# revdotcom/paper_accurate_fast_cheap

Measured on AMD Instinct MI355X. Metric: audio-sec/sec (1/RTF) GigaSpeech long-form encode, higher is better.
Workload: dtype f32+bf16-slot

## Files before the change

### include/pafc_encoder_ops.h

```cpp
#ifndef PAFC_ENCODER_OPS_H
#define PAFC_ENCODER_OPS_H

#include "pafc_wkv6.h"

#ifdef __cplusplus
extern "C" {
#endif

int pafc_dwconv1d_cl(int dtype, int B, int T_in, int C, int K, int left_pad, int T_out, const void *x,
                     const void *w, const void *bias, void *y, int glu, const int32_t *lens,
                     pafc_stream_t stream);

int pafc_dwconv1d_cl_ex(int dtype, int B, int T_in, int C, int K, int left_pad, int T_out, const void *x, long ldx,
                        const void *w, const void *bias, void *y, int act, const int32_t *lens, pafc_stream_t stream);

int pafc_dwconv1d_cl_ln_silu(int dtype, int B, int T_in, int C, int K, int left_pad, int T_out, const void *x, long ldx,
                             const void *w, const void *bias, const void *gamma, const void *beta, float eps, void *y,
                             const int32_t *lens, pafc_stream_t stream);

size_t pafc_dwconv1d_cl_wgrad_workspace_bytes(int B, int T_out, int C, int K);
int pafc_dwconv1d_cl_wgrad(int dtype, int B, int T_in, int C, int K, int left_pad, int T_out, const void *x, long ldx,
                           const void *dy, float *dw, float *dbias, void *workspace, size_t workspace_bytes,
                           pafc_stream_t stream);

int pafc_add_layernorm(int dtype, int dtype_out, int rows, int C, const void *x, const void *y, float alpha,
                       const int32_t *lens, int T, int mask_y, void *x_out, const void *gamma1, const void *beta1,
                       void *out1, long ld1, int silu1, int zero1, const void *gamma2, const void *beta2, void *out2,
                       long ld2, float eps, pafc_stream_t stream);

int pafc_add_layernorm_ex(int dtype, int dtype_out, int dtype_out2, int rows, int C, const void *x, const void *y, float alpha,
                          const int32_t *lens, int T, int mask_y, void *x_out, const void *gamma1, const void *beta1,
                          void *out1, long ld1, int silu1, int zero1, const void *gamma2, const void *beta2, void *out2,
                          long ld2, float eps, float *stats_x, float *stats_out1, pafc_stream_t stream);
int pafc_gemm_bf16_ph_ln(long M, int N, int K, const void *A, long lda, const void *W, long ldw, const void *bias,
                         const void *residual, long ldr, void *out, long ldo, float alpha, int act, int ln_mode, float *stats,
                         const float *csum, int ln_c, float ln_eps, int tile_m, pafc_stream_t stream);

int pafc_split_planes(long rows, int cols, const float *x, long ldx, void *out, long ldo, long lo_off, int triple,
                      pafc_stream_t stream);

size_t pafc_layernorm_bwd_workspace_bytes(long rows, int C);
int pafc_layernorm_bwd(int dtype_x, int dtype_dy, long rows, int C, const void *x, const void *dy, const void *gamma,
                       float eps, void *dx, float *dgamma_dbeta, void *workspace, size_t workspace_bytes,
                       pafc_stream_t stream);
int pafc_layernorm_bwd_add(int dtype_x, int dtype_dy, long rows, int C, const void *x, const void *dy, const void *gamma, float eps,
                           const void *dx_add, void *dx, float *dgamma_dbeta, void *workspace, size_t workspace_bytes,
                           pafc_stream_t stream);
// ... 183 lines not shown
```

### paper_accurate_fast_cheap_amd/_lib.py

```python
import ctypes
import os
from ctypes import c_float, c_int, c_long, c_size_t, c_ulonglong, c_void_p

import torch

_HERE = os.path.dirname(os.path.abspath(__file__))
SO_PATH = os.path.join(_HERE, "libpafc_hip.so")

PAFC_F32, PAFC_BF16 = 0, 1
_ERRORS = {
    -1: "null pointer", -2: "bad dims (B, T, C, H must be positive and C == H * 64)", -3: "head size must be 64",
    -4: "workspace too small", -5: "kernel launch failed", -6: "unsupported dtype", -7: "unsupported",
    -8: "r, k, v, w, y must be 16-byte aligned",
}


class PafcError(RuntimeError):
    pass


_lib = None


def lib():
# ... 12 lines not shown
            "(python -m paper_accurate_fast_cheap_amd.csrc.build). There is no CPU fallback.")
    from .csrc import build as _build
    if _build.built_key() != _build.source_key():
        raise PafcError(
            f"{SO_PATH} was not built from the sources in this tree (libpafc_hip.so.json: {_build.built_key()}, sources: "
            f"{_build.source_key()}): rebuild with python -m paper_accurate_fast_cheap_amd.csrc.build")
    _lib = _bind(ctypes.CDLL(SO_PATH))
    return _lib


P, I, G, Z, F, U = c_void_p, c_int, c_long, c_size_t, c_float, c_ulonglong
SIGNATURES = {
    "pafc_mha_rows": (I, [I, I, I, I, P, G, P, P, G, P, P, P, I, P, G, P]),
    "pafc_logp_gather_rows": (I, [I, G, I, P, G, P, P, P]),
    "pafc_mha_band": (I, [I, I, I, I, I, I, I, P, G, P, P, G, P, G, P, P, P, G, P]),
    "pafc_mha_rows_lse": (I, [I, I, I, I, P, G, P, P, G, P, P, P, I, P, G, P, P]),
    "pafc_mha_rows_bwd_workspace_bytes": (Z, [G, I]),
    "pafc_mha_rows_bwd": (I, [I, I, I, I, G, P, G, P, P, G, P, G, P, G, P, P, P, P, I, P, G, P, P, G, P, Z, P]),
    "pafc_lsm_loss_rows": (I, [I, G, I, P, G, P, F, P, P, P, P]),
    "pafc_lsm_loss_rows_bwd": (I, [I, G, I, P, G, P, F, P, P, P, G, P]),
    "pafc_mha_band_lse": (I, [I, I, I, I, I, I, I, P, G, P, P, G, P, G, P, P, P, G, P, P]),
    "pafc_mha_band_bwd_workspace_bytes": (Z, [I, I, I]),
    "pafc_mha_band_bwd": (I, [I, I, I, I, I, I, I, P, G, P, P, G, P, G, P, P, P, G, P, G, P, P, G, P, P, G, P, G, P, P, P, Z,
                              P]),
    "pafc_mha_step": (I, [I, I, I, I, I, I, P, G, P, P, P, P, P, G, P]),
    "pafc_attn_beam_select_workspace_bytes": (Z, [I, I]),
    "pafc_attn_beam_select": (I, [I, I, I, I, I, I, I, P, G, P, P, P, P, P, P, P, P, P, P, Z, P]),
    "pafc_mha_step_paths": (I, [I, I, I, I, I, I, P, G, P, P, G, P, P, P, P, G, P]),
    "pafc_joint_candidates": (I, [I, I, I, I, I, I, F, P, P, P, P, P, P, P]),
    "pafc_joint_frame": (I, [P, I, I, I, P, G, P, P, I, P]),
    "pafc_joint_collect": (I, [P, P, P, P, P, P, P, P]),
    "pafc_dwconv1d_cl": (I, [I, I, I, I, I, I, I, P, P, P, P, I, P, P]),
    "pafc_dwconv1d_cl_ex": (I, [I, I, I, I, I, I, I, P, G, P, P, P, I, P, P]),
    "pafc_dwconv1d_cl_ln_silu": (I, [I, I, I, I, I, I, I, P, G, P, P, P, P, F, P, P, P]),
    "pafc_dwconv1d_cl_wgrad_workspace_bytes": (Z, [I, I, I, I]),
    "pafc_dwconv1d_cl_wgrad": (I, [I, I, I, I, I, I, I, P, G, P, P, P, P, Z, P]),
    "pafc_add_layernorm": (I, [I, I, I, I, P, P, F, P, I, I, P, P, P, P, G, I, I, P, P, P, G, F, P]),
    "pafc_add_layernorm_ex": (I, [I, I, I, I, I, P, P, F, P, I, I, P, P, P, P, G, I, I, P, P, P, G, F, P, P, P]),
    "pafc_gemm_bf16_ph_ln": (I, [G, I, I, P, G, P, G, P, P, G, P, G, F, I, I, P, P, I, F, I, P]),
    "pafc_split_planes": (I, [G, I, P, G, P, G, G, I, P]),
    "pafc_layernorm_bwd_workspace_bytes": (Z, [G, I]),
    "pafc_layernorm_bwd": (I, [I, I, G, I, P, P, P, F, P, P, P, Z, P]),
    "pafc_layernorm_bwd_add": (I, [I, I, G, I, P, P, P, F, P, P, P, P, Z, P]),
    "pafc_layernorm_silu_fwd": (I, [I, I, G, I, P, P, P, F, P, P]),
    "pafc_layernorm_silu_bwd": (I, [I, I, G, I, P, P, P, P, F, P, P, P, Z, P]),
    "pafc_gemm_skinny_bf16": (I, [G, I, I, I, P, G, G, P, G, G, P, G, P, G, G, P, G, G, F, I, P, I, P, F, P, P]),
    "pafc_gemm_skinny_bf16_ex": (I, [G, I, I, I, P, G, G, P, G, G, P, G, P, G, G, P, G, G, F, I, I, P, I, I, P, F, P, P, P, I,
        P, P, F, P]),
    "pafc_decay_lora_skinny_bf16": (I, [G, I, I, P, G, P, P, P, P, G, P]),
    "pafc_tmix_shift_mix": (I, [I, I, I, I, I, I, P, P, P, P, P]),
    "pafc_tmix_mix4": (I, [I, I, I, I, I, I, P, P, P, P, P]),
    "pafc_tmix_lora_mix4_bf16": (I, [I, I, I, I, I, P, P, P, P, P, P]),
    "pafc_tmix_lora_down_bf16": (I, [I, I, I, I, I, I, P, P, P, P, P]),
    "pafc_tmix_shift_mix_prev": (I, [I, I, I, I, I, I, P, P, P, P, P, P]),
    "pafc_tmix_lora_mix4_bf16_prev": (I, [I, I, I, I, I, P, P, P, P, P, P, P]),
    "pafc_tmix_lora_down_bf16_prev": (I, [I, I, I, I, I, I, P, P, P, P, P, P]),
    "pafc_decay_lora_bf16": (I, [G, I, I, I, P, P, P, P, P, P]),
    "pafc_tmix_bwd_workspace_bytes": (Z, [G, I]),
    "pafc_tmix_shift_mix_bwd": (I, [I, I, I, I, I, P, P, P, P, P, P, Z, P]),
    "pafc_tmix_mix4_bwd": (I, [I, I, I, I, I, P, P, P, P, P, P, P, P, P, P, P, Z, P]),
    "pafc_tmix_mix4_bwd_rows": (I, [I, I, I, I, I, P, P, P, P, P, P, P, P, P, P, P, Z, P]),
    "pafc_conv3x3s2_nhwc_bf16": (I, [I, I, I, I, I, P, P, P, P, I, P]),
    "pafc_conv3x3s2_c1_nhwc_bf16": (I, [I, I, I, I, P, P, P, P, I, P]),
    "pafc_conv3x3s2_c1_wgrad_workspace_bytes": (Z, [I, I, I]),
    "pafc_conv3x3s2_c1_wgrad_bf16": (I, [I, I, I, I, P, P, P, P, P, Z, P]),
    "pafc_conv3x3s2_c1_nhwc_f32split": (I, [I, I, I, I, P, P, P, P, P, I, P]),
# ... 154 lines not shown
```

### paper_accurate_fast_cheap_amd/csrc/dwconv.hip

```cpp
#include <stdlib.h>
#include "pafc_common.h"
#include "../../include/pafc_encoder_ops.h"

namespace pafc {
namespace {

constexpr int KMAX = 31;
constexpr int TO = 16;

template <typename ET> struct Pair;
template <> struct Pair<float> {
    __device__ static __forceinline__ float2 load(const float *p) { return *reinterpret_cast<const float2 *>(p); }
    __device__ static __forceinline__ void store(float *p, float2 v) { *reinterpret_cast<float2 *>(p) = v; }
    __device__ static __forceinline__ float round(float v) { return v; }
};
template <> struct Pair<bf16_t> {
    __device__ static __forceinline__ float2 load(const bf16_t *p) {
        const uint32_t q = *reinterpret_cast<const uint32_t *>(p);
        return make_float2(bf16_bits_to_f32(q & 0xffffu), __uint_as_float(q & 0xffff0000u));
    }
    __device__ static __forceinline__ void store(bf16_t *p, float2 v) {
        *reinterpret_cast<uint32_t *>(p) = f32_to_bf16_bits(v.x) | (f32_to_bf16_bits(v.y) << 16);
    }
    __device__ static __forceinline__ float round(float v) { return round_bf16(v); }
};

__device__ __forceinline__ float sigmoidf_(float x) { return 1.f / (1.f + __expf(-x)); }

struct LnTail {
    const void *gamma, *beta;
    float eps;
};

// ... 85 lines not shown
        const float inv_c = 1.f / (float)C;
        float mean[TO];
#pragma unroll
        for (int o = 0; o < TO; ++o) {
            mean[o] = tot[o] * inv_c;
            const float d0 = u0[o] - mean[o], d1 = u1[o] - mean[o];
            sv[o] = fmaf(d1, d1, d0 * d0);
        }
        __syncthreads();
        block_sums(sv);
        const float2 gv = Pair<ET>::load((const ET *)ln.gamma + c), bt = Pair<ET>::load((const ET *)ln.beta + c);
#pragma unroll
        for (int o = 0; o < TO; ++o) {
            const float rstd = rsqrtf(tot[o] * inv_c + ln.eps);
            float o0 = Pair<ET>::round(fmaf((u0[o] - mean[o]) * rstd, gv.x, bt.x));
            float o1 = Pair<ET>::round(fmaf((u1[o] - mean[o]) * rstd, gv.y, bt.y));
            o0 = o0 * sigmoidf_(o0);
            o1 = o1 * sigmoidf_(o1);
            if (t0 + o < T_out) Pair<ET>::store(yb + (size_t)(t0 + o) * C, make_float2(o0, o1));
        }
        return;
    }
#pragma unroll
    for (int o = 0; o < TO; ++o) {
        if (ACT == 2) {
            const float u0 = Pair<ET>::round(a0[o]), u1 = Pair<ET>::round(a1[o]);
            a0[o] = u0 * sigmoidf_(u0);
            a1[o] = u1 * sigmoidf_(u1);
        }
        if (t0 + o < T_out) Pair<ET>::store(yb + (size_t)(t0 + o) * C, make_float2(a0[o], a1[o]));
    }
}

template <typename ET, int K>
int launch(int B, int T_in, int C, int left_pad, int T_out, const void *x, long ldx, const void *w, const void *bias,
           void *y, int act, const int32_t *lens, const LnTail &ln, hipStream_t s) {
    dim3 grid((T_out + TO - 1) / TO, (C / 2 + 255) / 256, B), block(256);
    if (act == 1)
        hipLaunchKernelGGL((dwconv_kernel<ET, K, 1>), grid, block, 0, s, T_in, C, left_pad, T_out, (const ET *)x, ldx,
                           (const ET *)w, (const ET *)bias, (ET *)y, lens, ln);
    else if (act == 2)
        hipLaunchKernelGGL((dwconv_kernel<ET, K, 2>), grid, block, 0, s, T_in, C, left_pad, T_out, (const ET *)x, ldx,
                           (const ET *)w, (const ET *)bias, (ET *)y, lens, ln);
    else if (act == 3) {
        if constexpr (K == 31 || K == 15) {
            hipLaunchKernelGGL((dwconv_kernel<ET, K, 3>), grid, block, 0, s, T_in, C, left_pad, T_out, (const ET *)x, ldx,
                               (const ET *)w, (const ET *)bias, (ET *)y, lens, ln);
        } else {
            return PAFC_ERR_UNSUPPORTED;
        }
    } else
        hipLaunchKernelGGL((dwconv_kernel<ET, K, 0>), grid, block, 0, s, T_in, C, left_pad, T_out, (const ET *)x, ldx,
                           (const ET *)w, (const ET *)bias, (ET *)y, lens, ln);
    return hipGetLastError() == hipSuccess ? PAFC_OK : PAFC_ERR_LAUNCH;
}

template <typename ET>
int dispatch_k(int K, int B, int T_in, int C, int left_pad, int T_out, const void *x, long ldx, const void *w,
               const void *bias, void *y, int act, const int32_t *lens, const LnTail &ln, hipStream_t s) {
    switch (K) {
        case 31: return launch<ET, 31>(B, T_in, C, left_pad, T_out, x, ldx, w, bias, y, act, lens, ln, s);
        case 15: return launch<ET, 15>(B, T_in, C, left_pad, T_out, x, ldx, w, bias, y, act, lens, ln, s);
        case 7: return launch<ET, 7>(B, T_in, C, left_pad, T_out, x, ldx, w, bias, y, act, lens, ln, s);
        case 4: return launch<ET, 4>(B, T_in, C, left_pad, T_out, x, ldx, w, bias, y, act, lens, ln, s);
        case 3: return launch<ET, 3>(B, T_in, C, left_pad, T_out, x, ldx, w, bias, y, act, lens, ln, s);
        default: return PAFC_ERR_UNSUPPORTED;
    }
}


constexpr int WG_SPAN = 8 * TO;

template <typename ET, int K>
__global__ __launch_bounds__(256) void dwconv_wgrad_kernel(int T_in, int C, int left_pad, int T_out,
                                                           const ET *__restrict__ x, long ldx,
                                                           const ET *__restrict__ dy, float *__restrict__ part) {
    const int c = (blockIdx.y * 256 + threadIdx.x) * 2;
    if (c >= C) return;
    const int b = blockIdx.z;
    const ET *xb = x + (size_t)b * T_in * ldx;
    const ET *db = dy + (size_t)b * T_out * C;
    float a0[K], a1[K], s0 = 0.f, s1 = 0.f;
#pragma unroll
    for (int k = 0; k < K; ++k) a0[k] = a1[k] = 0.f;
    constexpr int NR = TO + K - 1;
    for (int t0 = blockIdx.x * WG_SPAN; t0 < min(T_out, (int)(blockIdx.x + 1) * WG_SPAN); t0 += TO) {
        float2 g[TO], in[NR];
#pragma unroll
        for (int o = 0; o < TO; ++o) {
            const int t = min(t0 + o, T_out - 1);
            g[o] = Pair<ET>::load(db + (size_t)t * C + c);
            if (t0 + o >= T_out) g[o] = make_float2(0.f, 0.f);
            s0 += g[o].x;
            s1 += g[o].y;
        }
#pragma unroll
        for (int q = 0; q < NR; ++q) {
            const int s = t0 - left_pad + q;
// ... 42 lines not shown
    return hipGetLastError() == hipSuccess ? PAFC_OK : PAFC_ERR_LAUNCH;
}

template <typename ET>
int dispatch_wgrad(int K, int B, int T_in, int C, int left_pad, int T_out, const void *x, long ldx, const void *dy,
                   float *part, float *dw, float *dbias, hipStream_t s) {
    switch (K) {
        case 31: return launch_wgrad<ET, 31>(B, T_in, C, left_pad, T_out, x, ldx, dy, part, dw, dbias, s);
        case 15: return launch_wgrad<ET, 15>(B, T_in, C, left_pad, T_out, x, ldx, dy, part, dw, dbias, s);
        case 7: return launch_wgrad<ET, 7>(B, T_in, C, left_pad, T_out, x, ldx, dy, part, dw, dbias, s);
        case 4: return launch_wgrad<ET, 4>(B, T_in, C, left_pad, T_out, x, ldx, dy, part, dw, dbias, s);
        case 3: return launch_wgrad<ET, 3>(B, T_in, C, left_pad, T_out, x, ldx, dy, part, dw, dbias, s);
        default: return PAFC_ERR_UNSUPPORTED;
    }
}

}
}

extern "C" int pafc_dwconv1d_cl(int dtype, int B, int T_in, int C, int K, int left_pad, int T_out, const void *x,
                                const void *w, const void *bias, void *y, int glu, const int32_t *lens,
                                pafc_stream_t stream) {
    if (!x || !w || !y) return PAFC_ERR_NULL_POINTER;
    if (B <= 0 || T_in <= 0 || T_out <= 0 || C <= 0 || (C % 2) || K <= 0 || K > pafc::KMAX || left_pad < 0 ||
        B > 65535)
        return PAFC_ERR_BAD_DIMS;
    return pafc_dwconv1d_cl_ex(dtype, B, T_in, C, K, left_pad, T_out, x, glu ? 2L * C : (long)C, w, bias, y, glu ? 1 : 0, lens,
                               stream);
}

extern "C" int pafc_dwconv1d_cl_ex(int dtype, int B, int T_in, int C, int K, int left_pad, int T_out, const void *x, long ldx,
                                   const void *w, const void *bias, void *y, int act, const int32_t *lens,
                                   pafc_stream_t stream) {
    if (!x || !w || !y) return PAFC_ERR_NULL_POINTER;
    if (B <= 0 || T_in <= 0 || T_out <= 0 || C <= 0 || (C % 2) || K <= 0 || K > pafc::KMAX || left_pad < 0 ||
        B > 65535 || act < 0 || act > 2 || ldx < (act == 1 ? 2L * C : (long)C) || (ldx % 2))
        return PAFC_ERR_BAD_DIMS;
    hipStream_t s = (hipStream_t)stream;
    const pafc::LnTail none{nullptr, nullptr, 0.f};
    if (dtype == PAFC_BF16)
        return pafc::dispatch_k<pafc::bf16_t>(K, B, T_in, C, left_pad, T_out, x, ldx, w, bias, y, act, lens, none, s);
    if (dtype == PAFC_F32) return pafc::dispatch_k<float>(K, B, T_in, C, left_pad, T_out, x, ldx, w, bias, y, act, lens, none, s);
    return PAFC_ERR_DTYPE;
}

extern "C" int pafc_dwconv1d_cl_ln_silu(int dtype, int B, int T_in, int C, int K, int left_pad, int T_out, const void *x, long ldx,
                                        const void *w, const void *bias, const void *gamma, const void *beta, float eps, void *y,
                                        const int32_t *lens, pafc_stream_t stream) {
    if (!x || !w || !y || !gamma || !beta) return PAFC_ERR_NULL_POINTER;
    if (B <= 0 || T_in <= 0 || T_out <= 0 || left_pad < 0 || B > 65535 || ldx < C || (ldx % 2)) return PAFC_ERR_BAD_DIMS;
    if (C != 512 || (K != 31 && K != 15)) return PAFC_ERR_UNSUPPORTED;
    if (dtype != PAFC_BF16) return PAFC_ERR_DTYPE;
    const pafc::LnTail ln{gamma, beta, eps};
    return pafc::dispatch_k<pafc::bf16_t>(K, B, T_in, C, left_pad, T_out, x, ldx, w, bias, y, 3, lens, ln, (hipStream_t)stream);
}

extern "C" size_t pafc_dwconv1d_cl_wgrad_workspace_bytes(int B, int T_out, int C, int K) {
    if (B <= 0 || T_out <= 0 || C <= 0 || K <= 0) return 0;
    return (size_t)B * ((T_out + pafc::WG_SPAN - 1) / pafc::WG_SPAN) * (K + 1) * C * sizeof(float);
}

extern "C" int pafc_dwconv1d_cl_wgrad(int dtype, int B, int T_in, int C, int K, int left_pad, int T_out, const void *x,
                                      long ldx, const void *dy, float *dw, float *dbias, void *workspace,
                                      size_t workspace_bytes, pafc_stream_t stream) {
    if (!x || !dy || !dw || !workspace) return PAFC_ERR_NULL_POINTER;
    if (B <= 0 || T_in <= 0 || T_out <= 0 || C <= 0 || (C % 2) || K <= 0 || K > pafc::KMAX || left_pad < 0 ||
        B > 65535 || ldx < C || (ldx % 2))
        return PAFC_ERR_BAD_DIMS;
    if (workspace_bytes < pafc_dwconv1d_cl_wgrad_workspace_bytes(B, T_out, C, K)) return PAFC_ERR_WORKSPACE;
    hipStream_t s = (hipStream_t)stream;
    float *part = (float *)workspace;
    if (dtype == PAFC_BF16)
        return pafc::dispatch_wgrad<pafc::bf16_t>(K, B, T_in, C, left_pad, T_out, x, ldx, dy, part, dw, dbias, s);
    if (dtype == PAFC_F32) return pafc::dispatch_wgrad<float>(K, B, T_in, C, left_pad, T_out, x, ldx, dy, part, dw, dbias, s);
    return PAFC_ERR_DTYPE;
}
```

### paper_accurate_fast_cheap_amd/hip_ops.py

```python
import contextlib
import ctypes
import math
import os
import threading
import weakref
from typing import List, Optional

import torch

from . import _lib
from ._lib import c_int, c_void_p
from .utils import graph_step


DISPATCH = dict(skinny_max_rows=640, own_gemm_min_rows=1, lds_resident_min_rows=8192, split_gemm_min_rows=1024,
                ln_fold_min_rows=24576, dwconv_ln_silu_max_rows=24575, split_small_max_rows=8192, split_layers_min_rows=256,
                ktail_min_k=2048)


def _load_dispatch():
    legacy = dict(skinny_max_rows="PAFC_SKINNY_MAX_ROWS", own_gemm_min_rows="PAFC_OWN_GEMM_MIN_ROWS",
                  lds_resident_min_rows="PAFC_LDS_RESIDENT_MIN_ROWS", split_gemm_min_rows="PAFC_SPLIT_GEMM_MIN_ROWS")
    for name, env in legacy.items():
        if os.environ.get(env):
            DISPATCH[name] = int(os.environ[env])
    for item in filter(None, os.environ.get("PAFC_DISPATCH", "").split(",")):
        name, _, value = item.partition("=")
        if name.strip() not in DISPATCH:
            raise ValueError(f"PAFC_DISPATCH: unknown threshold {name!r} (known: {sorted(DISPATCH)})")
        DISPATCH[name.strip()] = int(value)


_load_dispatch()


def train_gemms_own() -> bool:
    return os.environ.get("PAFC_TRAIN_OWN_GEMMS", "1") != "0"


def train_kernels_enabled() -> bool:
    import os
    return os.environ.get("PAFC_TRAIN_KERNELS", "1") != "0"


def _conv_rows_ld(x: torch.Tensor, who: str) -> int:
    if not x.is_cuda:
        raise _lib.PafcError("this op runs on the MI355X only (tensor is on %s); there is no CPU fallback" % x.device)
    if x.is_contiguous():
        return x.shape[-1]
    if x.dim() != 3 or x.stride(2) != 1 or x.stride(0) != x.shape[1] * x.stride(1) or x.stride(1) < x.shape[2] or x.stride(1) % 2 \
            or x.data_ptr() % (2 * x.element_size()):
        raise _lib.PafcError(f"{who}: x (B, T, C) with unit channel stride, rows of one even stride, an aligned channel pair")
    return x.stride(1)


def depthwise_conv1d_cl(x: torch.Tensor, weight: torch.Tensor, bias: Optional[torch.Tensor], left_pad: int,
                        out_len: int, glu: bool = False, lens: Optional[torch.Tensor] = None) -> torch.Tensor:
    _lib.require_gpu(weight, bias, lens)
    ldx = _conv_rows_ld(x, "depthwise_conv1d_cl")
    B, T, Cx = x.shape
    C = Cx // 2 if glu else Cx
    K = weight.shape[-1]
    if weight.shape != (C, 1, K) or weight.dtype != x.dtype or (bias is not None and bias.dtype != x.dtype):
        raise _lib.PafcError("depthwise weight must be (C, 1, K) in the activation dtype")
    if lens is not None and lens.dtype != torch.int32:
        raise _lib.PafcError("lens must be int32")
    y = torch.empty(B, out_len, C, dtype=x.dtype, device=x.device)
    rc = _lib.lib().pafc_dwconv1d_cl_ex(_lib.dtype_code(x.dtype), B, T, C, K, left_pad, out_len, _lib.ptr(x), ldx,
                                        _lib.ptr(weight), _lib.ptr(bias), _lib.ptr(y), int(glu), _lib.ptr(lens),
                                        _lib.stream_of(x))
    _lib.check(rc, "pafc_dwconv1d_cl")
    return y


def dwconv_ln_silu_ok(x: torch.Tensor, weight: torch.Tensor) -> bool:
    return (x.numel() // x.shape[-1] <= DISPATCH["dwconv_ln_silu_max_rows"] and x.dtype == torch.bfloat16 and x.is_cuda
            and x.shape[-1] == 512 and weight.shape[-1] in (15, 31))


def depthwise_conv1d_cl_ln_silu(x: torch.Tensor, weight: torch.Tensor, bias: Optional[torch.Tensor], left_pad: int, out_len: int,
                                gamma: torch.Tensor, beta: torch.Tensor, eps: float, lens: Optional[torch.Tensor] = None):
    _lib.require_gpu(weight, bias, gamma, beta, lens)
    ldx = _conv_rows_ld(x, "depthwise_conv1d_cl_ln_silu")
    B, T, C = x.shape
    K = weight.shape[-1]
    if not dwconv_ln_silu_ok(x, weight) or weight.shape != (C, 1, K) or any(
            t is not None and (t.dtype != x.dtype or not t.is_contiguous()) for t in (weight, bias, gamma, beta)):
        raise _lib.PafcError("depthwise_conv1d_cl_ln_silu: bf16, C = 512, K in (15, 31), contiguous parameters in the activation dtype")
    if lens is not None and lens.dtype != torch.int32:
        raise _lib.PafcError("lens must be int32")
    L = _lib.lib()
    y = torch.empty(B, out_len, C, dtype=x.dtype, device=x.device)
    rc = L.pafc_dwconv1d_cl_ln_silu(_lib.dtype_code(x.dtype), B, T, C, K, left_pad, out_len, _lib.ptr(x), ldx, _lib.ptr(weight),
                                    _lib.ptr(bias), _lib.ptr(gamma), _lib.ptr(beta), float(eps), _lib.ptr(y), _lib.ptr(lens),
                                    _lib.stream_of(x))
    _lib.check(rc, "pafc_dwconv1d_cl_ln_silu")
    return y


def depthwise_conv1d_cl_wgrad(x: torch.Tensor, dy: torch.Tensor, K: int, left_pad: int, want_bias: bool = True):
    _lib.require_gpu(dy)
    ldx = _conv_rows_ld(x, "depthwise_conv1d_cl_wgrad")
# ... 3488 lines not shown
```

### paper_accurate_fast_cheap_amd/transformer/fused.py

```python
from typing import List, Optional, Tuple

import os

import torch
import torch.nn.functional as F
from torch import nn

from .. import hip_ops
from ..rwkv_v6.rwkv_wrapper import RWKV_TmixWrapper
from ..rwkv_v6.rwkv_wrapper_bidirectional import RWKV_TmixWrapper_bidirectional
from ..rwkv_v6.rwkv_wrapper_bidirectional_direction_dropout import (RWKV_TmixWrapper_bidirectional_direction_dropout,
                                                                     RWKV_TmixWrapper_bidirectional_direction_dropout_both)
from ..rwkv_v6.wkv6_op import wkv6_forward, wkv6_forward_bidir


_DIR_DROP_SLOTS = (RWKV_TmixWrapper_bidirectional_direction_dropout, RWKV_TmixWrapper_bidirectional_direction_dropout_both)
_RWKV_SLOTS = (RWKV_TmixWrapper, RWKV_TmixWrapper_bidirectional) + _DIR_DROP_SLOTS


def _fold_norm(w: torch.Tensor, b: Optional[torch.Tensor], norm: nn.LayerNorm, interleave: int = 0):
    wf = w.float()
    bf = (b.float() if b is not None else 0) + wf @ norm.bias.float()
    wp = (wf * norm.weight.float()).to(torch.bfloat16)
    if interleave:
# ... 10 lines not shown
        self.rwkv = type(slot) in _RWKV_SLOTS
        self.reverse0 = False
        if type(slot) in _DIR_DROP_SLOTS:
            fwd, bwd = slot.rwkv_wrapper_forward, slot.rwkv_wrapper_backward
            if slot.bi_active:
                self.blocks = [fwd.tmix_block, bwd.tmix_block]
            elif slot.alt_decoding and slot.layer_id % 2 == 1:
                self.blocks, self.reverse0 = [bwd.tmix_block], True
            else:
                self.blocks = [fwd.tmix_block]
            self.slot_bf16 = bool(fwd.do_bfloat16)
        elif isinstance(slot, RWKV_TmixWrapper_bidirectional):
            self.blocks = [slot.rwkv_wrapper_forward.tmix_block, slot.rwkv_wrapper_backward.tmix_block]
        elif self.rwkv:
            self.blocks = [slot.tmix_block]
        else:
            self.blocks = []
        self.ndir = len(self.blocks)
        if type(slot) not in _DIR_DROP_SLOTS:
            self.slot_bf16 = bool(getattr(slot, "do_bfloat16", False))
        self._stamp = None
        self.refresh()

    def _current_stamp(self):
        ep = hip_ops.param_epoch()
        if getattr(self, "_stamp_params", None) is None or self._stamp_epoch != ep:
            L = self.layer
            ps = [p for b in self.blocks for p in b.parameters()] + [L.feed_forward_macaron.w_2.bias, L.feed_forward.w_2.bias,
                                                                        L.conv_module.pointwise_conv1.weight,
                                                                        L.conv_module.pointwise_conv1.bias,
                                                                        L.feed_forward_macaron.w_1.weight, L.feed_forward_macaron.w_2.weight,
                                                                        L.feed_forward.w_1.weight, L.feed_forward.w_2.weight,
                                                                        L.conv_module.pointwise_conv2.weight,
                                                                        L.norm_ff_macaron.weight, L.norm_ff_macaron.bias, L.norm_ff.weight,
                                                                        L.norm_ff.bias, L.norm_conv.weight, L.norm_conv.bias,
                                                                        L.feed_forward_macaron.w_1.bias, L.feed_forward.w_1.bias]
            self._stamp_params = [p for p in ps if p is not None]
            self._stamp_epoch = ep
        return (ep,) + tuple((p.data_ptr(), p._version, p.dtype) for p in self._stamp_params)

    def refresh(self):
        stamp = self._current_stamp()
        if stamp == self._stamp:
            self._fill.use()
            return
        bl = self.blocks
        with torch.no_grad():
            if self.rwkv:
                self._refresh_rwkv(bl)
            L = self.layer
            self.b2_macaron = (L.feed_forward_macaron.w_2.bias * L.ff_scale).contiguous()
            self.b2 = (L.feed_forward.w_2.bias * L.ff_scale).contiguous()
            pw1 = L.conv_module.pointwise_conv1
            self.pw1_glu = None
            rows2 = pw1.weight.shape[0]
            if pw1.weight.dtype == torch.bfloat16 and pw1.weight.is_cuda and rows2 % 128 == 0 \
                    and pw1.weight.shape[1] % 64 == 0:
                self.pw1_glu = {h: (hip_ops.glu_interleave(pw1.weight.squeeze(-1), h),
                                    hip_ops.glu_interleave(pw1.bias, h) if pw1.bias is not None else None)
                                for h in ((64, 32) if rows2 % 256 == 0 else (64,))}
            self._refresh_split()
            self._refresh_lnfold()
        self._stamp = stamp
        self._fill = hip_ops.DerivedFill()

    def _refresh_lnfold(self):
        L = self.layer
        self.lnf = None
        w1 = L.feed_forward.w_1.weight
        cm = L.conv_module
        if not (self.rwkv and w1.dtype == torch.bfloat16 and w1.is_cuda and L.size == 512 and L.feed_forward_macaron is not None
                and cm is not None and cm.pointwise_conv1.weight.shape[0] % 256 == 0 and cm.lorder == 0
                and os.environ.get("PAFC_LN_FOLD", "1") != "0"):
            return
        pw1 = cm.pointwise_conv1
        self.lnf = dict(ffm=_fold_norm(L.feed_forward_macaron.w_1.weight, L.feed_forward_macaron.w_1.bias, L.norm_ff_macaron),
                        ff=_fold_norm(L.feed_forward.w_1.weight, L.feed_forward.w_1.bias, L.norm_ff),
                        pw1=_fold_norm(pw1.weight.squeeze(-1), pw1.bias, L.norm_conv, interleave=32))

    def carry_folds(self):
        if getattr(self, "_carry_folds", None) is not None and self._carry_folds[0] == self._stamp:
            self._carry_folds[2].use()
            return self._carry_folds[1]
        L = self.layer
        folds = dict(ff=_fold_norm(L.feed_forward.w_1.weight, L.feed_forward.w_1.bias, L.norm_ff) + (L.norm_ff.eps,))
        if self.rwkv:
            folds["out"] = _fold_norm(self.Wo, None, self.blocks[0].ln_x) + (self.blocks[0].ln_x.eps,)
        self._carry_folds = (self._stamp, folds, hip_ops.DerivedFill())
        return folds

    def _refresh_split(self):
        L = self.layer
        self.split = None
        w1 = L.feed_forward.w_1.weight
        cm = L.conv_module
        if not (self.rwkv and self.slot_bf16 and w1.dtype == torch.float32 and w1.is_cuda and L.size % 128 == 0
                and w1.shape[0] % 128 == 0 and cm is not None and cm.pointwise_conv1.weight.shape[0] % 256 == 0):
            return
        sp = hip_ops.split_planes
        pw1 = cm.pointwise_conv1
        self.split = dict(
            ffm_w1=sp(L.feed_forward_macaron.w_1.weight.contiguous(), True), ffm_w2=sp(L.feed_forward_macaron.w_2.weight.contiguous(), True),
            ff_w1=sp(L.feed_forward.w_1.weight.contiguous(), True), ff_w2=sp(L.feed_forward.w_2.weight.contiguous(), True),
            pw1=sp(hip_ops.glu_interleave(pw1.weight.squeeze(-1), 32).contiguous(), True),
            pw1_b=hip_ops.glu_interleave(pw1.bias, 32).contiguous() if pw1.bias is not None else None,
            pw1_plain=sp(pw1.weight.squeeze(-1).contiguous(), True),
            pw2=sp(cm.pointwise_conv2.weight.squeeze(-1).contiguous(), True))

    def _refresh_rwkv(self, bl):
        self.maa_x = [b.time_maa_x.reshape(-1).contiguous() for b in bl]
        self.maa_x_n = torch.stack(self.maa_x).contiguous()
        self.W1 = torch.stack([b.time_maa_rkvw_w1 for b in bl]).contiguous()
        self.W1n = torch.stack([b.time_maa_rkvw_w1.t() for b in bl]).contiguous()
        self.D1n = torch.stack([b.time_decay_w1.t() for b in bl]).contiguous()
        self.W2 = [b.time_maa_rkvw_w2.contiguous() for b in bl]
        self.W2t = torch.stack([b.time_maa_rkvw_w2.transpose(1, 2) for b in bl]).contiguous()
        self.maa4 = torch.stack([torch.stack([b.time_maa_r.reshape(-1), b.time_maa_k.reshape(-1),
                                              b.time_maa_v.reshape(-1), b.time_maa_w.reshape(-1)])
                                 for b in bl]).contiguous()
        self.Wrkv = torch.stack([getattr(b, n).weight.t() for n in ("receptance", "key", "value") for b in bl]
                                ).contiguous()
        self.Wrkv_n = torch.stack([getattr(b, n).weight for n in ("receptance", "key", "value") for b in bl]
                                  ).contiguous()
        self.D2n = torch.stack([b.time_decay_w2.t() for b in bl]).contiguous()
        self.D1 = torch.stack([b.time_decay_w1 for b in bl]).contiguous()
        self.D2 = torch.stack([b.time_decay_w2 for b in bl]).contiguous()
        self.time_decay = torch.stack([b.time_decay.reshape(1, -1) for b in bl]).contiguous()
        self.u = [b.time_faaaa.contiguous() for b in bl]
        wo = torch.cat([b.output.weight for b in bl], dim=1)
        self.Wo = (wo * 0.5 if self.ndir == 2 else wo).contiguous()


def _layer_shape_common(layer: nn.Module) -> bool:
    cm = layer.conv_module
    return (layer.normalize_before and layer.feed_forward_macaron is not None and cm is not None
            and cm.use_layer_norm and isinstance(cm.activation, nn.SiLU)
            and isinstance(layer.feed_forward.activation, nn.SiLU)
            and isinstance(layer.feed_forward_macaron.activation, nn.SiLU))


# ... 225 lines not shown
    xo = x2.view(B, T, C)
    if next_fold:
        stn = new_stats()
        return _ln(L.norm_final, xo, want_x=False, stats_out1=stn)[1], stn
    return _final_norms(L, xo, next_norm)


_SPLIT_GEMM_MIN_ROWS = hip_ops.DISPATCH["split_layers_min_rows"]


def split_eligible(plan: LayerPlan, x: torch.Tensor) -> bool:
    return (plan.split is not None and x.dtype == torch.float32 and x.is_cuda
            and x.numel() // x.shape[-1] >= _SPLIT_GEMM_MIN_ROWS)


def layer_forward_split(plan: LayerPlan, x: torch.Tensor, hp: torch.Tensor, lens: Optional[torch.Tensor],
                        next_norm: Optional[nn.LayerNorm], next_split: bool):
    L, S = plan.layer, plan.split
    B, T, C = x.shape
    M = B * T
    masked = lens is not None
    cm = L.conv_module
    G = hip_ops.gemm_ph_ex
    x = _ffn_split(L.feed_forward_macaron, S["ffm_w1"], S["ffm_w2"], hp, x, L.ff_scale, plan.b2_macaron, inplace=False)
    h = _ln(L.norm_mha, x, out_dtype=torch.bfloat16, want_x=False)[1]
    x = slot_forward(plan, h, residual=x)
    hc = _ln(L.norm_conv, x, zero_rows=masked, lens=lens, T=T, want_x=False, split1=True)[1]
    hc, left_pad, Tc = _causal_pad(cm, hc, T)
    if B * Tc <= hip_ops._SPLIT_SMALL_MAX_ROWS and B * Tc * 2 * C <= (1 << 22):
        p = G(hc.view(B * Tc, 2 * C), S["pw1_plain"], cm.pointwise_conv1.bias, a_split=True, out_kind="f32").view(B, Tc, 2 * C)
        dw = hip_ops.depthwise_conv1d_cl(p, cm.depthwise_conv.weight, cm.depthwise_conv.bias, left_pad, T, glu=True)
    else:
        p = G(hc.view(B * Tc, 2 * C), S["pw1"], S["pw1_b"], "glu", a_split=True, out_kind="f32").view(B, Tc, C)
        dw = hip_ops.depthwise_conv1d_cl(p, cm.depthwise_conv.weight, cm.depthwise_conv.bias, left_pad, T)
    g = _ln(cm.norm, dw, silu=True, split1=True)[1]
    if not masked:
        x2 = x.view(M, C)
        G(g.view(M, 2 * C), S["pw2"], cm.pointwise_conv2.bias, residual=x2, out=x2, a_split=True, out_kind="f32")
        h2 = _ln(L.norm_ff, x, want_x=False, split1=True)[1]
    else:
        c = G(g.view(M, 2 * C), S["pw2"], cm.pointwise_conv2.bias, a_split=True, out_kind="f32").view(B, T, C)
        x, h2, _ = _ln(L.norm_ff, x, c, lens=lens, T=T, mask_y=True, split1=True)
    x = _ffn_split(L.feed_forward, S["ff_w1"], S["ff_w2"], h2, x, L.ff_scale, plan.b2, inplace=True)
    return _final_norms(L, x, next_norm, split_next=next_split)


def _carry_slot_ok(slot: nn.Module) -> bool:
    if type(slot) is RWKV_TmixWrapper:
        return bool(slot.do_bfloat16)
    from .mamba2 import MambaAttWrapper
    if type(slot) is MambaAttWrapper and slot.streamable:
        m = slot.mamba
        return bool(m.fused_inference and m.ssd_kernel and m.d_state == 128 and m.d_inner <= 1024
                    and m.conv1d.weight.dtype == torch.bfloat16 and m.in_proj.weight.dtype == torch.bfloat16)
    return False


def carry_eligible(layer: nn.Module, x: torch.Tensor) -> bool:
    cm = layer.conv_module
    return (_layer_shape_common(layer) and _carry_slot_ok(layer.self_attn) and cm.lorder > 0 and cm.kernel_size <= 31
            and layer.size % 64 == 0 and layer.size <= 1024 and x.is_cuda and x.dtype == torch.bfloat16)


def _chunk_slot_rwkv(plan: LayerPlan, h: torch.Tensor, x: torch.Tensor, shift: torch.Tensor, s_in: Optional[torch.Tensor], *,
                     sk: bool, in_place: bool, out: Optional[torch.Tensor] = None):
    B, T, C = h.shape
    M = B * T
# ... 221 lines not shown
```

Before: 48830.

## Add persistent software-pipelined f32 depthwise conv kernel with transposed taps

Adds a persistent depthwise-conv kernel for f32 K=31 with no activation. Each block loops over strided time tiles and prefetches the next tile's input rows into registers while computing the current one. The grid is sized to the CU count, and tiles are partitioned into groups. Weights can be supplied pre-transposed as (K, C), which allows coalesced float2 tap loads; the layer plan caches this transpose. The large register footprint (31 taps ×2 plus 46 rows of float2) risks spills or low occupancy, and the kernel is enabled by default, with an env var to turn it off.

```diff
diff --git a/include/pafc_encoder_ops.h b/include/pafc_encoder_ops.h
--- a/include/pafc_encoder_ops.h
+++ b/include/pafc_encoder_ops.h
@@ -13,6 +13,10 @@
 
 int pafc_dwconv1d_cl_ex(int dtype, int B, int T_in, int C, int K, int left_pad, int T_out, const void *x, long ldx,
                         const void *w, const void *bias, void *y, int act, const int32_t *lens, pafc_stream_t stream);
+
+int pafc_dwconv1d_cl_tw(int dtype, int B, int T_in, int C, int K, int left_pad, int T_out, const void *x, long ldx,
+                        const void *w, const void *wt, const void *bias, void *y, int act, const int32_t *lens,
+                        pafc_stream_t stream);
 
 int pafc_dwconv1d_cl_ln_silu(int dtype, int B, int T_in, int C, int K, int left_pad, int T_out, const void *x, long ldx,
                              const void *w, const void *bias, const void *gamma, const void *beta, float eps, void *y,
diff --git a/paper_accurate_fast_cheap_amd/_lib.py b/paper_accurate_fast_cheap_amd/_lib.py
--- a/paper_accurate_fast_cheap_amd/_lib.py
+++ b/paper_accurate_fast_cheap_amd/_lib.py
@@ -68,6 +68,7 @@
     "pafc_joint_collect": (I, [P, P, P, P, P, P, P, P]),
     "pafc_dwconv1d_cl": (I, [I, I, I, I, I, I, I, P, P, P, P, I, P, P]),
     "pafc_dwconv1d_cl_ex": (I, [I, I, I, I, I, I, I, P, G, P, P, P, I, P, P]),
+    "pafc_dwconv1d_cl_tw": (I, [I, I, I, I, I, I, I, P, G, P, P, P, P, I, P, P]),
     "pafc_dwconv1d_cl_ln_silu": (I, [I, I, I, I, I, I, I, P, G, P, P, P, P, F, P, P, P]),
     "pafc_dwconv1d_cl_wgrad_workspace_bytes": (Z, [I, I, I, I]),
     "pafc_dwconv1d_cl_wgrad": (I, [I, I, I, I, I, I, I, P, G, P, P, P, P, Z, P]),
diff --git a/paper_accurate_fast_cheap_amd/csrc/dwconv.hip b/paper_accurate_fast_cheap_amd/csrc/dwconv.hip
--- a/paper_accurate_fast_cheap_amd/csrc/dwconv.hip
+++ b/paper_accurate_fast_cheap_amd/csrc/dwconv.hip
@@ -1,4 +1,5 @@
 #include <stdlib.h>
+#include <type_traits>
 #include "pafc_common.h"
 #include "../../include/pafc_encoder_ops.h"
 
@@ -150,9 +151,142 @@
     }
 }
 
+__device__ __forceinline__ float2 dw_load_row(const float *xb, long xc, int c, int T_in, int s) {
+    const int sc = min(max(s, 0), T_in - 1);
+    return Pair<float>::load(xb + (size_t)sc * xc + c);
+}
+
+template <int K, int NPF, bool WT>
+__global__ __launch_bounds__(256, 2) void dwconv_pipe_kernel(int T_in, int C, int left_pad, int T_out, const float *__restrict__ x,
+                                                             long ldx, const float *__restrict__ w, const float *__restrict__ wt,
+                                                             const float *__restrict__ bias, float *__restrict__ y,
+                                                             const int32_t *__restrict__ lens, int groups) {
+    constexpr int NR = TO + K - 1, NA = NPF;
+    static_assert(NPF >= 0 && NPF <= NR, "rows ahead");
+    const int c = (blockIdx.y * 256 + threadIdx.x) * 2;
+    if (c >= C) return;
+    const int b = blockIdx.z;
+    const int ntiles = (T_out + TO - 1) / TO;
+    const int grp = blockIdx.x % groups, stride = ((int)gridDim.x - grp + groups - 1) / groups;
+    const int hi = (int)((long)ntiles * (grp + 1) / groups);
+    int tile = (int)((long)ntiles * grp / groups) + blockIdx.x / groups;
+    if (tile >= hi) return;
+    const float *xb = x + (size_t)b * T_in * ldx;
+    float *yb = y + (size_t)b * T_out * C + c;
+    const int valid = lens ? min(T_in, lens[b]) : T_in;
+
+    float w0[K], w1[K];
+    if constexpr (WT) {
+#pragma unroll
+        for (int k = 0; k < K; ++k) {
+            const float2 t = Pair<float>::load(wt + (size_t)k * C + c);
+            w0[k] = t.x;
+            w1[k] = t.y;
+        }
+    } else {
+#pragma unroll
+        for (int k = 0; k < K; ++k) {
+            w0[k] = w[(size_t)c * K + k];
+            w1[k] = w[(size_t)(c + 1) * K + k];
+        }
+    }
+    float2 bv = make_float2(0.f, 0.f);
+    if (bias) bv = Pair<float>::load(bias + c);
+
+    float2 in[NR];
+#pragma unroll
+    for (int q = 0; q < NR; ++q) in[q] = dw_load_row(xb, ldx, c, T_in, tile * TO - left_pad + q);
+
+    auto body = [&](auto has_next) {
+        constexpr bool NEXT = decltype(has_next)::value;
+        const int t0 = tile * TO, s0 = t0 - left_pad, n0 = s0 + stride * TO;
+        auto row = [&](int q) {
+            const int s = s0 + q;
+            return (s >= 0 && s < valid) ? in[q] : make_float2(0.f, 0.f);
+        };
+        float2 ahead[NA > 0 ? NA : 1];
+        if constexpr (NEXT && NA > 0) {
+#pragma unroll
+            for (int q = 0; q < NA; ++q) {
+                ahead[q] = row(q);
+                in[q] = dw_load_row(xb, ldx, c, T_in, n0 + q);
+                __builtin_amdgcn_sched_barrier(0);
+            }
+        }
+        float a0[TO], a1[TO];
+#pragma unroll
+        for (int o = 0; o < TO; ++o) { a0[o] = bv.x; a1[o] = bv.y; }
+#pragma unroll
+        for (int q = 0; q < NR; ++q) {
+            const float2 v = (NEXT && q < NA) ? ahead[q] : row(q);
+#pragma unroll
+            for (int o = 0; o < TO; ++o) {
+                const int k = q - o;
+                if (k >= 0 && k < K) {
+                    a0[o] = fmaf(w0[k], v.x, a0[o]);
+                    a1[o] = fmaf(w1[k], v.y, a1[o]);
+                }
+            }
+        }
+        if constexpr (NEXT) {
+#pragma unroll
+            for (int q = NA; q < NR; ++q) in[q] = dw_load_row(xb, ldx, c, T_in, n0 + q);
+            __builtin_amdgcn_sched_barrier(0);
+        }
+        if constexpr (!NEXT) {
+#pragma unroll
+            for (int o = 0; o < TO; ++o) asm volatile("" : "+v"(a0[o]), "+v"(a1[o]));
+        }
+#pragma unroll
+        for (int o = 0; o < TO; ++o)
+            if (NEXT || t0 + o < T_out) Pair<float>::store(yb + (size_t)(t0 + o) * C, make_float2(a0[o], a1[o]));
+    };
+    if (tile + stride < hi) {
+        __builtin_amdgcn_s_waitcnt(0x0F70);
+        do {
+            body(std::true_type{});
+            tile += stride;
+        } while (tile + stride < hi);
+    }
+    body(std::false_type{});
+}
+
+bool dwconv_pipe() {
+    const char *e = getenv("PAFC_DWCONV_PIPE");
+    return !(e && e[0] == '0');
+}
+
+constexpr int PIPE_ROWS_AHEAD = 28;
+constexpr int PIPE_BLOCKS_PER_CU = 2;
+
+template <int K>
+int launch_pipe(int B, int T_in, int C, int left_pad, int T_out, const float *x, long ldx, const float *w, const float *wt,
+                const float *bias, float *y, const int32_t *lens, hipStream_t s) {
+    const int ntiles = (T_out + TO - 1) / TO, ycols = (C / 2 + 255) / 256;
+    long nblk = (long)device_cus() * PIPE_BLOCKS_PER_CU / ((long)B * ycols);
+    if (const char *e = getenv("PAFC_DWCONV_BLOCKS")) nblk = atol(e);
+    nblk = nblk < 1 ? 1 : (nblk > ntiles ? ntiles : nblk);
+    dim3 grid((unsigned)nblk, ycols, B), block(256);
+    int groups = nblk < 8 ? (int)nblk : 8;
+    if (const char *e = getenv("PAFC_DWCONV_GROUPS")) groups = atoi(e) < 1 ? 1 : (atoi(e) < nblk ? atoi(e) : (int)nblk);
+#define PAFC_DWPIPE_(NPF, WT) \
+    hipLaunchKernelGGL((dwconv_pipe_kernel<K, NPF, WT>), grid, block, 0, s, T_in, C, left_pad, T_out, x, ldx, w, wt, bias, y, lens, \
+                       groups)
+    if (wt) PAFC_DWPIPE_(PIPE_ROWS_AHEAD, true); else PAFC_DWPIPE_(PIPE_ROWS_AHEAD, false);
+#undef PAFC_DWPIPE_
+    return hipGetLastError() == hipSuccess ? PAFC_OK : PAFC_ERR_LAUNCH;
+}
+
 template <typename ET, int K>
-int launch(int B, int T_in, int C, int left_pad, int T_out, const void *x, long ldx, const void *w, const void *bias,
+int launch(int B, int T_in, int C, int left_pad, int T_out, const void *x, long ldx, const void *w, const void *wt, const void *bias,
            void *y, int act, const int32_t *lens, const LnTail &ln, hipStream_t s) {
+    if constexpr (sizeof(ET) == 4 && K == 31) {
+        if (act == 0) {
+            if (dwconv_pipe())
+                return launch_pipe<K>(B, T_in, C, left_pad, T_out, (const float *)x, ldx, (const float *)w, (const float *)wt,
+                                      (const float *)bias, (float *)y, lens, s);
+        }
+    }
     dim3 grid((T_out + TO - 1) / TO, (C / 2 + 255) / 256, B), block(256);
     if (act == 1)
         hipLaunchKernelGGL((dwconv_kernel<ET, K, 1>), grid, block, 0, s, T_in, C, left_pad, T_out, (const ET *)x, ldx,
@@ -174,14 +308,14 @@
 }
 
 template <typename ET>
-int dispatch_k(int K, int B, int T_in, int C, int left_pad, int T_out, const void *x, long ldx, const void *w,
+int dispatch_k(int K, int B, int T_in, int C, int left_pad, int T_out, const void *x, long ldx, const void *w, const void *wt,
                const void *bias, void *y, int act, const int32_t *lens, const LnTail &ln, hipStream_t s) {
     switch (K) {
-        case 31: return launch<ET, 31>(B, T_in, C, left_pad, T_out, x, ldx, w, bias, y, act, lens, ln, s);
-        case 15: return launch<ET, 15>(B, T_in, C, left_pad, T_out, x, ldx, w, bias, y, act, lens, ln, s);
-        case 7: return launch<ET, 7>(B, T_in, C, left_pad, T_out, x, ldx, w, bias, y, act, lens, ln, s);
-        case 4: return launch<ET, 4>(B, T_in, C, left_pad, T_out, x, ldx, w, bias, y, act, lens, ln, s);
-        case 3: return launch<ET, 3>(B, T_in, C, left_pad, T_out, x, ldx, w, bias, y, act, lens, ln, s);
+        case 31: return launch<ET, 31>(B, T_in, C, left_pad, T_out, x, ldx, w, wt, bias, y, act, lens, ln, s);
+        case 15: return launch<ET, 15>(B, T_in, C, left_pad, T_out, x, ldx, w, wt, bias, y, act, lens, ln, s);
+        case 7: return launch<ET, 7>(B, T_in, C, left_pad, T_out, x, ldx, w, wt, bias, y, act, lens, ln, s);
+        case 4: return launch<ET, 4>(B, T_in, C, left_pad, T_out, x, ldx, w, wt, bias, y, act, lens, ln, s);
+        case 3: return launch<ET, 3>(B, T_in, C, left_pad, T_out, x, ldx, w, wt, bias, y, act, lens, ln, s);
         default: return PAFC_ERR_UNSUPPORTED;
     }
 }
@@ -290,15 +424,22 @@
 extern "C" int pafc_dwconv1d_cl_ex(int dtype, int B, int T_in, int C, int K, int left_pad, int T_out, const void *x, long ldx,
                                    const void *w, const void *bias, void *y, int act, const int32_t *lens,
                                    pafc_stream_t stream) {
+    return pafc_dwconv1d_cl_tw(dtype, B, T_in, C, K, left_pad, T_out, x, ldx, w, nullptr, bias, y, act, lens, stream);
+}
+
+extern "C" int pafc_dwconv1d_cl_tw(int dtype, int B, int T_in, int C, int K, int left_pad, int T_out, const void *x, long ldx,
+                                   const void *w, const void *wt, const void *bias, void *y, int act, const int32_t *lens,
+                                   pafc_stream_t stream) {
     if (!x || !w || !y) return PAFC_ERR_NULL_POINTER;
     if (B <= 0 || T_in <= 0 || T_out <= 0 || C <= 0 || (C % 2) || K <= 0 || K > pafc::KMAX || left_pad < 0 ||
         B > 65535 || act < 0 || act > 2 || ldx < (act == 1 ? 2L * C : (long)C) || (ldx % 2))
         return PAFC_ERR_BAD_DIMS;
+    if (wt && dtype != PAFC_F32) return PAFC_ERR_DTYPE;
     hipStream_t s = (hipStream_t)stream;
     const pafc::LnTail none{nullptr, nullptr, 0.f};
     if (dtype == PAFC_BF16)
-        return pafc::dispatch_k<pafc::bf16_t>(K, B, T_in, C, left_pad, T_out, x, ldx, w, bias, y, act, lens, none, s);
-    if (dtype == PAFC_F32) return pafc::dispatch_k<float>(K, B, T_in, C, left_pad, T_out, x, ldx, w, bias, y, act, lens, none, s);
+        return pafc::dispatch_k<pafc::bf16_t>(K, B, T_in, C, left_pad, T_out, x, ldx, w, nullptr, bias, y, act, lens, none, s);
+    if (dtype == PAFC_F32) return pafc::dispatch_k<float>(K, B, T_in, C, left_pad, T_out, x, ldx, w, wt, bias, y, act, lens, none, s);
     return PAFC_ERR_DTYPE;
 }
 
@@ -310,7 +451,7 @@
     if (C != 512 || (K != 31 && K != 15)) return PAFC_ERR_UNSUPPORTED;
     if (dtype != PAFC_BF16) return PAFC_ERR_DTYPE;
     const pafc::LnTail ln{gamma, beta, eps};
-    return pafc::dispatch_k<pafc::bf16_t>(K, B, T_in, C, left_pad, T_out, x, ldx, w, bias, y, 3, lens, ln, (hipStream_t)stream);
+    return pafc::dispatch_k<pafc::bf16_t>(K, B, T_in, C, left_pad, T_out, x, ldx, w, nullptr, bias, y, 3, lens, ln, (hipStream_t)stream);
 }
 
 extern "C" size_t pafc_dwconv1d_cl_wgrad_workspace_bytes(int B, int T_out, int C, int K) {
diff --git a/paper_accurate_fast_cheap_amd/hip_ops.py b/paper_accurate_fast_cheap_amd/hip_ops.py
--- a/paper_accurate_fast_cheap_amd/hip_ops.py
+++ b/paper_accurate_fast_cheap_amd/hip_ops.py
@@ -54,9 +54,14 @@
     return x.stride(1)
 
 
+def dwconv_taps_t(weight: torch.Tensor) -> torch.Tensor:
+    return weight.squeeze(1).t().contiguous()
+
+
 def depthwise_conv1d_cl(x: torch.Tensor, weight: torch.Tensor, bias: Optional[torch.Tensor], left_pad: int,
-                        out_len: int, glu: bool = False, lens: Optional[torch.Tensor] = None) -> torch.Tensor:
-    _lib.require_gpu(weight, bias, lens)
+                        out_len: int, glu: bool = False, lens: Optional[torch.Tensor] = None,
+                        taps_t: Optional[torch.Tensor] = None) -> torch.Tensor:
+    _lib.require_gpu(weight, bias, lens, taps_t)
     ldx = _conv_rows_ld(x, "depthwise_conv1d_cl")
     B, T, Cx = x.shape
     C = Cx // 2 if glu else Cx
@@ -65,9 +70,11 @@
         raise _lib.PafcError("depthwise weight must be (C, 1, K) in the activation dtype")
     if lens is not None and lens.dtype != torch.int32:
         raise _lib.PafcError("lens must be int32")
+    if taps_t is not None and (glu or x.dtype != torch.float32 or taps_t.dtype != torch.float32 or taps_t.shape != (K, C)):
+        raise _lib.PafcError("taps_t must be the float32 (K, C) transpose of the weight, for float32 inputs without glu")
     y = torch.empty(B, out_len, C, dtype=x.dtype, device=x.device)
-    rc = _lib.lib().pafc_dwconv1d_cl_ex(_lib.dtype_code(x.dtype), B, T, C, K, left_pad, out_len, _lib.ptr(x), ldx,
-                                        _lib.ptr(weight), _lib.ptr(bias), _lib.ptr(y), int(glu), _lib.ptr(lens),
+    rc = _lib.lib().pafc_dwconv1d_cl_tw(_lib.dtype_code(x.dtype), B, T, C, K, left_pad, out_len, _lib.ptr(x), ldx,
+                                        _lib.ptr(weight), _lib.ptr(taps_t), _lib.ptr(bias), _lib.ptr(y), int(glu), _lib.ptr(lens),
                                         _lib.stream_of(x))
     _lib.check(rc, "pafc_dwconv1d_cl")
     return y
diff --git a/paper_accurate_fast_cheap_amd/transformer/fused.py b/paper_accurate_fast_cheap_amd/transformer/fused.py
--- a/paper_accurate_fast_cheap_amd/transformer/fused.py
+++ b/paper_accurate_fast_cheap_amd/transformer/fused.py
@@ -66,6 +66,7 @@
                                                                         L.feed_forward_macaron.w_1.weight, L.feed_forward_macaron.w_2.weight,
                                                                         L.feed_forward.w_1.weight, L.feed_forward.w_2.weight,
                                                                         L.conv_module.pointwise_conv2.weight,
+                                                                        L.conv_module.depthwise_conv.weight,
                                                                         L.norm_ff_macaron.weight, L.norm_ff_macaron.bias, L.norm_ff.weight,
                                                                         L.norm_ff.bias, L.norm_conv.weight, L.norm_conv.bias,
                                                                         L.feed_forward_macaron.w_1.bias, L.feed_forward.w_1.bias]
@@ -126,6 +127,7 @@
     def _refresh_split(self):
         L = self.layer
         self.split = None
+        self.dw_taps_t = None
         w1 = L.feed_forward.w_1.weight
         cm = L.conv_module
         if not (self.rwkv and self.slot_bf16 and w1.dtype == torch.float32 and w1.is_cuda and L.size % 128 == 0
@@ -140,6 +142,8 @@
             pw1_b=hip_ops.glu_interleave(pw1.bias, 32).contiguous() if pw1.bias is not None else None,
             pw1_plain=sp(pw1.weight.squeeze(-1).contiguous(), True),
             pw2=sp(cm.pointwise_conv2.weight.squeeze(-1).contiguous(), True))
+        if cm.depthwise_conv.weight.dtype == torch.float32:
+            self.dw_taps_t = hip_ops.dwconv_taps_t(cm.depthwise_conv.weight)
 
     def _refresh_rwkv(self, bl):
         self.maa_x = [b.time_maa_x.reshape(-1).contiguous() for b in bl]
@@ -431,7 +435,7 @@
         dw = hip_ops.depthwise_conv1d_cl(p, cm.depthwise_conv.weight, cm.depthwise_conv.bias, left_pad, T, glu=True)
     else:
         p = G(hc.view(B * Tc, 2 * C), S["pw1"], S["pw1_b"], "glu", a_split=True, out_kind="f32").view(B, Tc, C)
-        dw = hip_ops.depthwise_conv1d_cl(p, cm.depthwise_conv.weight, cm.depthwise_conv.bias, left_pad, T)
+        dw = hip_ops.depthwise_conv1d_cl(p, cm.depthwise_conv.weight, cm.depthwise_conv.bias, left_pad, T, taps_t=plan.dw_taps_t)
     g = _ln(cm.norm, dw, silu=True, split1=True)[1]
     if not masked:
         x2 = x.view(M, C)
```

Measured after the change: 49040, median of 6. Within noise of the previous version (+0.4%).
